# Grice-Lab/HmmUFOtu

Measured on AMD Instinct MI355X. Metric: reads placed/sec (whole node), gg_97_otus GTR+dGamma 250bp; HBM GB/s %peak, higher is better.
Workload: dtype f64

## Files before the change

hmmufotu_amd/csrc/hu_engine.hip:

```cpp
#include <algorithm>
#include <cmath>
#include <cstdio>
#include <cstring>
#include <limits>
#include <map>
#include <atomic>
#include <thread>
#include <memory>
#include <mutex>
#include <chrono>
#include <fstream>
#include <sstream>
#include <new>
#include <stdexcept>
#include "hu_common.h"
#include "hu_kern_sep.h"
#include "hu_kern_align.h"
#include "hu_kern_tree.h"
#include "hu_kern_blk.h"
#include "hu_kern_refsort.h"
#include "hu_kern_rank.h"
#include "hu_kern_anneal.h"
#include "hu_kern_build.h"
#include "hu_kern_otucs.h"
// ... 1112 lines not shown
typedef HuPlaceRec HostPlace;

struct HuKnobs {
	int viterbi_hbm = 0;
	int viterbi_values = 0;
	int viterbi_mode = 0;
	int viterbi_dec1 = 0;
	int vw_diag = 0;
	int viterbi_force_redo = 0;
	int tile_unsorted = 0;
	int pairs32 = 0;
	int topk_fast_min = 16384;
	int topk_general = 0;
	int scan_pairs = 0;
	int streaming_sep = 0;
	int est_unsorted = 0, place_unsorted = 0;
	int xcd_map = 1;
	int est_var = 0, place_var = 0;
	int place_nosplit = 0;
	int place_lds_pad = 0;
	int est_lds_pad = 0;
	int vit_lds_pad = 0;
	int scan_lds_pad = 0;
	int trace = 0;
	int width_split = 1;
	int sort_seq = 0;
	int refsort_wgs = HU_RS_WGS_PER_CU * 256;
	int ref_nofuse = 0;
	int refsort_host = 0;
	int inject_fault = 0;
};
struct HuKnobEntry { const char* name; int HuKnobs::* field; };
static const HuKnobEntry kKnobs[] = {
	{"viterbi_hbm", &HuKnobs::viterbi_hbm}, {"viterbi_values", &HuKnobs::viterbi_values}, {"viterbi_mode", &HuKnobs::viterbi_mode},
	{"viterbi_dec1", &HuKnobs::viterbi_dec1}, {"vw_diag", &HuKnobs::vw_diag}, {"viterbi_force_redo", &HuKnobs::viterbi_force_redo},
	{"pairs32", &HuKnobs::pairs32}, {"tile_unsorted", &HuKnobs::tile_unsorted}, {"topk_fast_min", &HuKnobs::topk_fast_min}, {"scan_pairs", &HuKnobs::scan_pairs}, {"topk_general", &HuKnobs::topk_general}, {"streaming_sep", &HuKnobs::streaming_sep},
	{"est_unsorted", &HuKnobs::est_unsorted}, {"place_unsorted", &HuKnobs::place_unsorted}, {"xcd_map", &HuKnobs::xcd_map},
	{"est_var", &HuKnobs::est_var}, {"place_var", &HuKnobs::place_var}, {"place_nosplit", &HuKnobs::place_nosplit}, {"width_split", &HuKnobs::width_split},
	{"place_lds_pad", &HuKnobs::place_lds_pad}, {"est_lds_pad", &HuKnobs::est_lds_pad}, {"vit_lds_pad", &HuKnobs::vit_lds_pad}, {"scan_lds_pad", &HuKnobs::scan_lds_pad}, {"trace", &HuKnobs::trace}, {"inject_fault", &HuKnobs::inject_fault}, {"refsort_host", &HuKnobs::refsort_host}, {"ref_nofuse", &HuKnobs::ref_nofuse}, {"refsort_wgs", &HuKnobs::refsort_wgs}, {"sort_seq", &HuKnobs::sort_seq},
};
static void knobs_from_env(HuKnobs& k) {
	for(const HuKnobEntry& e : kKnobs) {
		std::string env = "HU_";
		for(const char* c = e.name; *c; ++c) env += (char) toupper(*c);
		const char* v = getenv(env.c_str());
		if(!v) continue;
		char* end = nullptr;
		const long x = strtol(v, &end, 10);
		k.*(e.field) = (end == v) ? 1 : (int) x;
	}
}

enum { ST_NONE = 0, ST_READS = 1, ST_ALIGNED = 2, ST_SEEDED = 3, ST_ESTIMATED = 4, ST_FILTERED = 5, ST_PLACED = 6, ST_FINISHED = 7 };

struct hu_batch {
	hu_db* db = nullptr;
	int maxReads = 0, n = 0, nSeq = 0, state = ST_NONE;
	bool paired = false, fromCodes = false, profile = false;
	HuKnobs knob;
	int maxBases = 1 << 30;
	bool fixedRoot = false;
	bool placesGiven = false;
	bool pair16 = false;
	int scanWidth = 0;
	int pairsKind = 0;
	int seedCap = HU_MAX_SEEDS;
	hipStream_t stream = nullptr;
	hipEvent_t ev[2 * HU_T_COUNT];
	bool evSet[HU_T_COUNT] = {false};
	float ms[HU_T_COUNT];
	double wall[4] = {0, 0, 0, 0};
	DBuf<char> dBases, dTraces, dRows;
	DBuf<HuReadDesc> dDescs;
	DBuf<double> dScratch;
	DBuf<uint8_t> dDec;
	DBuf<HuVitOut> dVit;
	DBuf<HuAlnDev> dAlns;
	DBuf<int8_t> dCodes;
	DBuf<int32_t> dStart, dEnd, dSeedCnt, dSeedId, dGiven, dPermCnt;
	DBuf<uint16_t> dPerm;
	DBuf<uint32_t> dRp, dPairs, dSeedDN, dParDN, dBmin, dRSpan, dTileSpan;
	DBuf<int32_t> dTileQ, dSlotRead, dReadSlot;
	DBuf<uint32_t> dRq;
	DBuf<unsigned long long> dRefScratch;
	DBuf<int32_t> dHv, dZeroPar; DBuf<unsigned long long> dPairsC; int refHvCount = 0; double refHvHeight = NAN;
	DBuf<int32_t> dBail, dNanCnt, dNanId; DBuf<uint32_t> dNanDN;
	int nRefBail = 0;
	DBuf<uint32_t> dRefPiv; DBuf<unsigned long long> dRefL0; bool refFused = false;
	int refHostAll = 0;
	DBuf<int32_t> dIns, dTileIns, dRetry;
	DBuf<uint32_t> dSortK, dSortV;
	DBuf<uint32_t> dCsCnt;
	DBuf<HuEstOut> dEst;
	DBuf<HuCand> dCands;
	DBuf<HuPlaceOut> dPlaceOut;
	DBuf<int32_t> dCandCnt, dCandOff, dMeta;
	DBuf<uint8_t> dFiltSlot;
	DBuf<HuPlaceRec> dPlaces;
	DBuf<hu_place_rec> dBest;
	size_t nc = 0;
	int maxGapSites = 0, maxBaseSites = 0;
	bool hostCands = false;
	DBuf<double> dRootLL;
	PinnedVec<double> hRootLL;
// ... 183 lines not shown
		tr += rd.len + b->db->dev.K + 8;
	}
	int rc;
	if((rc = b->dBases.ensure(b->hBases.size() + 1)) != HU_OK) return rc;
	b->cellsTotal = cells; b->cornerTotal = corners;
	if((rc = b->dDec.ensure((size_t) decs + 1)) != HU_OK) return rc;
	if((rc = b->dTraces.ensure((size_t) tr + 1)) != HU_OK) return rc;
	if((rc = b->dVit.ensure(b->nSeq)) != HU_OK) return rc;
	if(!b->hBases.empty()) HIPCHK(hipMemcpyAsync(b->dBases.p, b->hBases.data(), b->hBases.size(), hipMemcpyHostToDevice, b->stream));
	if((rc = upload_descs(b)) != HU_OK) return rc;
	b->state = ST_READS;
	return HU_OK;
} catch(...) { return hu_catch_all("hu_batch_set_reads"); }

static int ensure_read_buffers(hu_batch* b) {
	const HuDbDev& d = b->db->dev;
	const size_t n = (size_t) b->n;
	const size_t tiles = (n + HU_READ_TILE - 1) / HU_READ_TILE;
	int rc;
	if((rc = b->dCodes.ensure(n * d.csLen)) != HU_OK) return rc;
	if((rc = b->dStart.ensure(n)) != HU_OK) return rc;
	if((rc = b->dEnd.ensure(n)) != HU_OK) return rc;
	if((rc = b->dRp.ensure(tiles * d.WQ * HU_READ_TILE * 16)) != HU_OK) return rc;
	if((rc = b->dTileQ.ensure(tiles * (d.WQ + 1))) != HU_OK) return rc;
	if((rc = b->dSlotRead.ensure(std::max<size_t>(tiles, 1) * HU_READ_TILE)) != HU_OK) return rc;
	if((rc = b->dReadSlot.ensure(std::max<size_t>(n, 1))) != HU_OK) return rc;
	if((rc = b->dRq.ensure(std::max<size_t>(n, 1) * ((d.WQ + 31) / 32))) != HU_OK) return rc;
	if((rc = b->dIns.ensure(std::max<size_t>(n, 1) * (HU_MAX_INS + 1))) != HU_OK) return rc;
	if((rc = b->dTileIns.ensure(std::max<size_t>(tiles, 1) * (HU_READ_TILE * HU_MAX_INS + 1))) != HU_OK) return rc;
	if((rc = b->dRSpan.ensure(std::max<size_t>(n, 1) * 2)) != HU_OK) return rc;
	if((rc = b->dTileSpan.ensure(std::max<size_t>(tiles, 1) * 2)) != HU_OK) return rc;
	return HU_OK;
}

static int order_by_key(hu_batch* b, const uint32_t* key, const uint32_t* val, size_t n, uint32_t bound, uint32_t* out, bool runsInOrder) {
	if(!n) return HU_OK;
	const size_t m = (size_t) bound + 1;
	int rc;
	const size_t nTiles = (m + 1023) / 1024;
	if((rc = b->dCsCnt.ensure(3 * m + nTiles + 8)) != HU_OK) return rc;
	uint32_t* cnt = b->dCsCnt.p; uint32_t* start = cnt + m; uint32_t* cur = start + m + 1; uint32_t* tiles = cur + m;
	HIPCHK(hipMemsetAsync(cnt, 0, m * 4, b->stream));
	k_cs_hist<<<(unsigned)((n + 255) / 256), 256, 0, b->stream>>>((int) n, key, bound, cnt);
	k_cs_tile_sums<<<(unsigned) nTiles, 1024, 0, b->stream>>>((int) m, cnt, tiles);
	k_cs_scan_tiles<<<1, 1024, 0, b->stream>>>((int) nTiles, tiles);
	k_cs_scan<<<(unsigned) nTiles, 1024, 0, b->stream>>>((int) m, cnt, tiles, start, cur);
	k_cs_scatter<<<(unsigned)((n + 255) / 256), 256, 0, b->stream>>>((int) n, key, val, bound, cur, out);
	if(runsInOrder) k_cs_runs<<<(unsigned)((m + 3) / 4), 256, 0, b->stream>>>((int) bound, start, out);
	HIPCHK(hipGetLastError());
	return HU_OK;
}

static int tile_reads(hu_batch* b, const HuAlnDev* alns) {
	const int n = b->n;
	if(!n) return HU_OK;
	const int tiles = (n + HU_READ_TILE - 1) / HU_READ_TILE;
	int rc;
	if((rc = b->dSortK.ensure((size_t) n * 2)) != HU_OK || (rc = b->dSortV.ensure((size_t) n * 2)) != HU_OK) return rc;
	k_tile_keys<<<(n + 255) / 256, 256, 0, b->stream>>>(n, alns, b->dStart.p, b->dEnd.p, b->dSortK.p, b->dSortV.p);
	if(b->knob.tile_unsorted) HIPCHK(hipMemcpyAsync(b->dSortV.p + n, b->dSortV.p, (size_t) n * 4, hipMemcpyDeviceToDevice, b->stream));
	else if((rc = order_by_key(b, b->dSortK.p, b->dSortV.p, (size_t) n, (uint32_t) b->db->dev.csLen + 1u, b->dSortV.p + n, true)) != HU_OK) return rc;
	k_tile_slots<<<(tiles * HU_READ_TILE + 255) / 256, 256, 0, b->stream>>>(n, tiles * HU_READ_TILE, b->dSortV.p + n, b->dSlotRead.p, b->dReadSlot.p);
	HIPCHK(hipGetLastError());
	return HU_OK;
}

static int set_aligned_impl(hu_batch* b, int n, const int8_t* codes, hipMemcpyKind kind, const int32_t* start, const int32_t* end, int maxBases = -1) {
	if(!b || n < 0 || n > b->maxReads || (n > 0 && (!codes || !start || !end))) { hu_set_error("hu_batch_set_aligned: bad argument"); return HU_ERR_ARG; }
	HIPCHK(hipSetDevice(b->db->device));
	const HuDbDev& d = b->db->dev;
	b->n = n; b->nSeq = n; b->paired = false; b->fromCodes = true;
	if(maxBases >= 0) b->maxBases = maxBases;
	else {
		int mb = 0;
		for(int r = 0; r < n; ++r) {
			if(!(start[r] >= 0 && start[r] <= end[r] && end[r] < d.csLen)) continue;
			const int8_t* c = codes + (size_t) r * d.csLen; int k = 0;
			for(int j = start[r]; j <= end[r]; ++j) k += c[j] >= 0;
			mb = std::max(mb, k);
		}
		b->maxBases = mb;
	}
	int rc;
	if((rc = ensure_read_buffers(b)) != HU_OK) return rc;
	b->hAlns.assign(n, HuAlnDev());
	b->hStart.assign(start, start + n); b->hEnd.assign(end, end + n);
	for(int r = 0; r < n; ++r) {
		HuAlnDev& a = b->hAlns[r];
		memset(&a, 0, sizeof(a));
		const bool ok = start[r] >= 0 && start[r] <= end[r] && end[r] < d.csLen && start[r] >= d.winStart && end[r] < d.winStart + d.winLen;
		a.status = ok ? HU_READ_OK : HU_READ_INVALID;
		a.csStart = start[r] + 1; a.csEnd = end[r] + 1;
		if(!ok) { b->hStart[r] = (int32_t) d.winStart; b->hEnd[r] = (int32_t) d.winStart - 1; }
	}
	(void) hipGetLastError();
	if(n) {
		if((const void*) codes != (const void*) b->dCodes.p) HIPCHK(hipMemcpyAsync(b->dCodes.p, codes, (size_t) n * d.csLen, kind, b->stream));
		HIPCHK(hipMemcpyAsync(b->dStart.p, b->hStart.data(), (size_t) n * 4, hipMemcpyHostToDevice, b->stream));
		HIPCHK(hipMemcpyAsync(b->dEnd.p, b->hEnd.data(), (size_t) n * 4, hipMemcpyHostToDevice, b->stream));
		const int tiles = (n + HU_READ_TILE - 1) / HU_READ_TILE;
		HIPCHK(hipMemsetAsync(b->dRp.p, 0, (size_t) tiles * d.WQ * HU_READ_TILE * 16 * 4, b->stream));
		if((rc = tile_reads(b, nullptr)) != HU_OK) return rc;
		k_planes_from_codes<<<n, 64, 0, b->stream>>>(d, b->dCodes.p, b->dStart.p, b->dEnd.p, b->dRp.p, b->dRq.p, b->dIns.p, b->dReadSlot.p, (uint2*) b->dRSpan.p);
		k_tile_lists<<<tiles, 64, 0, b->stream>>>(d, n, b->dRq.p, b->dIns.p, b->dTileQ.p, b->dTileIns.p, b->dSlotRead.p, (const uint2*) b->dRSpan.p, (uint2*) b->dTileSpan.p);
		HIPCHK(hipGetLastError());
	}
	b->state = ST_ALIGNED;
	return HU_OK;
}
extern "C" int hu_batch_set_aligned(hu_batch* b, int n, const int8_t* codes, const int32_t* start, const int32_t* end) try {
	return set_aligned_impl(b, n, codes, hipMemcpyHostToDevice, start, end);
} catch(...) { return hu_catch_all("hu_batch_set_aligned"); }

enum VitFill { VF_WAVE4, VF_WAVE4_DIAG1, VF_WAVE4_DIAG2, VF_WAVE8, VF_DEC2_256, VF_DEC2_512, VF_DEC, VF_VALUES, VF_HBM };
struct VitPlan {
	VitFill fill;
	size_t lds;
	int decRpl;
	bool wave() const { return fill <= VF_WAVE8; }
	bool dec() const { return fill <= VF_DEC; }
};
static VitPlan plan_viterbi(const HuKnobs& kb, int maxLen, size_t vlds, int haloW) {
	if(vlds > 96 * 1024 || kb.viterbi_hbm) return {VF_HBM, 0, 0};
	if(kb.viterbi_values) return {VF_VALUES, vlds, 0};
	const int mode = kb.viterbi_mode ? kb.viterbi_mode : (kb.viterbi_dec1 ? 1 : 0);
	if(mode == 0 && maxLen <= 512) {
		const size_t wl = (size_t) 3 * std::min(haloW, 512) * sizeof(double) + (size_t)(kb.vit_lds_pad > 0 && kb.vit_lds_pad <= 40 ? kb.vit_lds_pad : 0) * 1024;
		if(maxLen > 256) return {VF_WAVE8, wl, 8};
// ... 114 lines not shown
				if((rc = fillValues(b->dDescs.p, b->nSeq, b->dScratch.p, b->dVit.p, HU_READ_NEEDS_VALUES)) != HU_OK) return rc;
				HIPCHK(hipGetLastError());
				HIPCHK(hipMemcpyAsync(b->hVit.data(), b->dVit.p, (size_t) b->nSeq * sizeof(HuVitOut), hipMemcpyDeviceToHost, b->stream));
				HIPCHK(hu_wait(b->stream));
			}
		}
		std::vector<int> redo;
		for(int s = 0; s < b->nSeq; ++s) if(b->hVit[s].status == HU_READ_NEEDS_FULL && !(b->hDescs[s].nRegions == 1 && !b->hDescs[s].reg[0].band)) redo.push_back(s);
		auto fullDp = [&](HuReadDesc& rd) { build_regions(b->db, rd.len, nullptr, rd); return rd.scratchOff; };
		if((rc = redoChunked(redo, fullDp, 0)) != HU_OK) return rc;
		for(int s : redo) b->hDescs[s].nRegions = -1;
		if(kb.trace) {
			static const char* const fillName[] = {"k_viterbi_wave<4>", "k_viterbi_wave<4, 1>", "k_viterbi_wave<4, 2>", "k_viterbi_wave<8>", "k_viterbi_dec2<256>", "k_viterbi_dec2<512>", "k_viterbi_dec", "k_viterbi_lds", "k_viterbi"};
			fprintf(stderr, "[hu] align: %d sequences, longest %d, fill %s, %zu bytes of LDS, %zu redone for values, %zu by the full-DP fallback\n", b->nSeq, maxLen, fillName[vp.fill], vp.lds, nValues, redo.size());
		}
		for(int s = 0; s < b->nSeq; ++s) if(b->hVit[s].status == HU_READ_NEEDS_FULL) { b->hVit[s].status = HU_READ_INVALID; hostVit = true; }
		if(hostVit) HIPCHK(hipMemcpyAsync(b->dVit.p, b->hVit.data(), (size_t) b->nSeq * sizeof(HuVitOut), hipMemcpyHostToDevice, b->stream));
		{
			Timer t(b, HU_T_ALIGN_BUILD);
			k_align_rows<<<b->nSeq, 64, 0, b->stream>>>(d, b->dDescs.p, b->dBases.p, b->dTraces.p, b->dVit.p, b->dRows.p, b->dAlns.p);
			if(b->paired) k_merge_rows<<<b->n, 256, 0, b->stream>>>(d, b->n, o->ignore_orient, b->dRows.p, b->dAlns.p);
			const int tiles = (b->n + HU_READ_TILE - 1) / HU_READ_TILE;
			HIPCHK(hipMemsetAsync(b->dRp.p, 0, (size_t) tiles * d.WQ * HU_READ_TILE * 16 * 4, b->stream));
			if((rc = tile_reads(b, b->dAlns.p)) != HU_OK) return rc;
			k_encode_rows<<<b->n, 64, 0, b->stream>>>(d, b->dRows.p, b->dAlns.p, b->dCodes.p, b->dStart.p, b->dEnd.p, b->dRp.p, b->dRq.p, b->dIns.p, b->dReadSlot.p, (uint2*) b->dRSpan.p);
			k_tile_lists<<<tiles, 64, 0, b->stream>>>(d, b->n, b->dRq.p, b->dIns.p, b->dTileQ.p, b->dTileIns.p, b->dSlotRead.p, (const uint2*) b->dRSpan.p, (uint2*) b->dTileSpan.p);
		}
		HIPCHK(hipGetLastError());
		b->hAlns.resize(b->nSeq);
		b->hStart.resize(b->n); b->hEnd.resize(b->n);
		HIPCHK(hipMemcpyAsync(b->hAlns.data(), b->dAlns.p, (size_t) b->nSeq * sizeof(HuAlnDev), hipMemcpyDeviceToHost, b->stream));
		HIPCHK(hipMemcpyAsync(b->hStart.data(), b->dStart.p, (size_t) b->n * 4, hipMemcpyDeviceToHost, b->stream));
		HIPCHK(hipMemcpyAsync(b->hEnd.data(), b->dEnd.p, (size_t) b->n * 4, hipMemcpyDeviceToHost, b->stream));
		HIPCHK(hu_wait(b->stream));
		for(int s = 0; s < b->nSeq; ++s) b->hAlns[s].usedFull |= (b->hDescs[s].nRegions == -1 || (b->hDescs[s].nRegions == 1 && !b->hDescs[s].reg[0].band)) ? 1 : 0;
	}
	b->state = ST_ALIGNED;
	return HU_OK;
} catch(...) { return hu_catch_all("hu_align_batch"); }

__global__ void k_seed_drop_empty(int n, const int32_t* __restrict__ rstart, const int32_t* __restrict__ rend, int32_t* __restrict__ seedCnt);
static inline HuReadPlanes read_planes(const hu_batch* b) { return HuReadPlanes{b->dRp.p, b->dRq.p, b->dIns.p, b->dReadSlot.p, (const uint2*) b->dRSpan.p}; }


extern "C" int hu_sort_desc_device(int device, const double* keys, int rows, int n, int32_t* order) try {
	if(!keys || !order || rows < 1 || n < 0 || n > HU_MAX_SEEDS) { hu_set_error("hu_sort_desc_device: bad argument"); return HU_ERR_ARG; }
	if(hu_device_count() <= 0) { hu_set_error("no gfx950 device visible: the engine has no CPU path"); return HU_ERR_DEVICE; }
	HIPCHK(hipSetDevice(device));
	if(n == 0) return HU_OK;
	DBuf<double> dk; DBuf<int32_t> dor;
	int rc;
// ... 361 lines not shown
	uint32_t* bmin = nullptr;
	if(dOnly) {
		if((rc = b->dBmin.ensure(std::max<size_t>(n, 1) * nBlk + 16)) != HU_OK) return rc;
		if((rc = b->dRetry.ensure(n + 1)) != HU_OK) return rc;
		bmin = b->dBmin.p;
	}
	b->refFused = refOrder && n > 0 && ref_fused_l0(b, o, b->pair16);
	if(b->refFused) {
		if((rc = b->dRefPiv.ensure(n * 4)) != HU_OK || (rc = b->dRefL0.ensure(n * (size_t)(d.nNodesPad / 64) * 2)) != HU_OK) return rc;
		k_ref_pivots<<<(unsigned)((n + 63) / 64), 64, 0, b->stream>>>(d, read_planes(b), b->n, b->dRefPiv.p);
		HIPCHK(hipGetLastError());
	}
	uint32_t* stat = bmin && b->knob.trace ? bmin + n * nBlk : nullptr;
	if(stat) HIPCHK(hipMemsetAsync(stat, 0, 64, b->stream));
	(void) hipGetLastError();
	if(n) {
		const int tiles = (b->n + HU_READ_TILE - 1) / HU_READ_TILE;
		const dim3 grid(tiles, d.nNodesPad / 256);
		{
			Timer t(b, HU_T_SEED_PDIST);
			const dim3 grid4(tiles, (d.nNodesPad + 1023) / 1024);
			if(dOnly && narrow) k_seed_dscan4<uint8_t><<<grid4, 256, (size_t)(b->knob.scan_lds_pad > 0 && b->knob.scan_lds_pad <= 44 ? b->knob.scan_lds_pad : 0) * 1024, b->stream>>>(d, b->dRp.p, b->dTileQ.p, (uint8_t*) b->dPairs.p, b->dSlotRead.p, bmin, (const uint2*) b->dTileSpan.p);
			else if(dOnly) k_seed_dscan4<uint16_t><<<grid4, 256, 0, b->stream>>>(d, b->dRp.p, b->dTileQ.p, (uint16_t*) b->dPairs.p, b->dSlotRead.p, bmin, (const uint2*) b->dTileSpan.p);
			else if(b->refFused && b->pair16) k_seed_pdist2<uint16_t, true><<<grid, 256, 0, b->stream>>>(d, b->dRp.p, b->dTileQ.p, b->dTileIns.p, (uint16_t*) b->dPairs.p, b->dSlotRead.p, b->dRefPiv.p, b->dRefL0.p);
			else if(b->refFused) k_seed_pdist2<uint32_t, true><<<grid, 256, 0, b->stream>>>(d, b->dRp.p, b->dTileQ.p, b->dTileIns.p, b->dPairs.p, b->dSlotRead.p, b->dRefPiv.p, b->dRefL0.p);
			else if(b->pair16) k_seed_pdist2<uint16_t><<<grid, 256, 0, b->stream>>>(d, b->dRp.p, b->dTileQ.p, b->dTileIns.p, (uint16_t*) b->dPairs.p, b->dSlotRead.p);
			else k_seed_pdist2<uint32_t><<<grid, 256, 0, b->stream>>>(d, b->dRp.p, b->dTileQ.p, b->dTileIns.p, b->dPairs.p, b->dSlotRead.p);
		}
		{
			Timer t(b, HU_T_SEED_TOPK);
			if(dOnly) {
				int32_t* retry = b->dRetry.p;
				HIPCHK(hipMemsetAsync(retry, 0, 4, b->stream));
				#define TOPK_ARGS(T) d, (const T*) b->dPairs.p, bmin, read_planes(b), o->max_nseed, b->dSeedCnt.p, b->dSeedId.p, b->dSeedDN.p, b->dParDN.p, stat, retry
				if(narrow) { k_seed_topk_straight<uint8_t><<<b->n, 256, 0, b->stream>>>(TOPK_ARGS(uint8_t), b->knob.topk_general); k_seed_topk_d<uint8_t, true><<<std::min(b->n, 1024), 256, 0, b->stream>>>(TOPK_ARGS(uint8_t)); }
				else { k_seed_topk_straight<uint16_t><<<b->n, 256, 0, b->stream>>>(TOPK_ARGS(uint16_t), b->knob.topk_general); k_seed_topk_d<uint16_t, true><<<std::min(b->n, 1024), 256, 0, b->stream>>>(TOPK_ARGS(uint16_t)); }
				#undef TOPK_ARGS
			}
			else if(refOrder) { if((rc = seed_order_libstdcxx_device(b, o)) != HU_OK) return rc; }
			else {
				if(b->pair16) k_seed_topk<uint16_t><<<b->n, 256, 0, b->stream>>>(d, (const uint16_t*) b->dPairs.p, o->max_height, o->max_nseed, b->dSeedCnt.p, b->dSeedId.p, b->dSeedDN.p, b->knob.topk_fast_min);
				else k_seed_topk<uint32_t><<<b->n, 256, 0, b->stream>>>(d, b->dPairs.p, o->max_height, o->max_nseed, b->dSeedCnt.p, b->dSeedId.p, b->dSeedDN.p, b->knob.topk_fast_min);
				k_parent_pairs<<<((unsigned) n * HU_MAX_SEEDS + 255) / 256, 256, 0, b->stream>>>(d, b->n, b->dPairs.p, b->pair16 ? 1 : 0, b->dSeedCnt.p, b->dSeedId.p, b->dParDN.p);
			}
		}
		k_seed_drop_empty<<<(b->n + 255) / 256, 256, 0, b->stream>>>(b->n, b->dStart.p, b->dEnd.p, b->dSeedCnt.p);
		HIPCHK(hipGetLastError());
		if(stat) {
			uint32_t h[16];
			HIPCHK(hipMemcpyAsync(h, stat, 64, hipMemcpyDeviceToHost, b->stream)); HIPCHK(hu_wait(b->stream));
// ... 1233 lines not shown
```

hmmufotu_amd/csrc/hu_kern_align.h:

```cpp
#pragma once
#include "hu_common.h"

struct HuVitOut { int32_t alnStart, alnEnd, alnFrom, alnTo, traceLen, status; double minScore; };

__device__ inline bool reg_contains(const HuRegion& g, int i, int j) {
	if(j < g.j0 || j > g.j1 || i < g.i0 || i > g.i1) return false;
	if(g.band) { int dist = (i - g.from) - (j - g.start); if(!(dist <= g.nIns && dist >= -g.nDel)) return false; }
	return true;
}

struct VitCtx {
	const HuReadDesc* rd;
	const double* scr;
	double tNN, tNB;
};

__device__ inline void vit_lookup(const VitCtx& c, int upto, int i, int j, double& m, double& ii, double& d) {
	const HuReadDesc& rd = *c.rd;
	for(int r = upto - 1; r >= 0; --r) {
		const HuRegion& g = rd.reg[r];
		if(reg_contains(g, i, j)) {
			const int64_t idx = (g.off + (int64_t)(j - g.j0) * (g.i1 - g.i0 + 1) + (i - g.i0)) * 3;
			m = c.scr[idx]; ii = c.scr[idx + 1]; d = c.scr[idx + 2];
			return;
// ... 996 lines not shown
		}
		ok = (st == HU_READ_OK);
		if(ok) {
			if(b.seqStart < a.seqStart) a.seqStart = b.seqStart;
			if(b.seqEnd > a.seqEnd) a.seqEnd = b.seqEnd;
			if(b.hmmStart < a.hmmStart) a.hmmStart = b.hmmStart;
			if(b.hmmEnd > a.hmmEnd) a.hmmEnd = b.hmmEnd;
			if(b.csStart < a.csStart) a.csStart = b.csStart;
			if(b.csEnd > a.csEnd) a.csEnd = b.csEnd;
			a.cost = a.cost + b.cost;
			a.usedFull |= b.usedFull;
		}
		a.status = st;
		alns[r] = a;
	}
	__syncthreads();
	if(!ok) return;
	char* ra = rows + (size_t) r * db.csLen;
	const char* rb = rows + (size_t)(n + r) * db.csLen;
	for(int c = threadIdx.x; c < db.csLen; c += 256) if(ra[c] == '.' && rb[c] != '.') ra[c] = rb[c];
}

__device__ inline void planes_of_codes(const HuDbDev& db, const int8_t* __restrict__ cd, int start, int end, int r, int slot, int lane,
		uint32_t* __restrict__ rp, uint32_t* __restrict__ rq, int32_t* __restrict__ ins, uint2* __restrict__ rspan) {
	const int tile = slot / HU_READ_TILE, t = slot % HU_READ_TILE;
	const int nw32 = (db.WQ + 31) / 32;
	uint32_t* qbits = rq + (size_t) r * nw32;
	int32_t* il = ins + (size_t) r * (HU_MAX_INS + 1);
	const int QM = (db.K + 127) / 128;
	int nIns = 0;
	for(int base = QM * 128; base < db.WQ * 128; base += 64) {
		const int c = db.posCol[base + lane];
		const bool in = c >= start && c <= end && cd[c >= 0 ? c : 0] >= 0 && c >= 0;
		nIns += __popcll(__ballot(in));
	}
	const bool dense = nIns > HU_MAX_INS;
	uint32_t acc = 0;
	int li = 0;
	uint32_t f1 = 0xffffu, l1 = 0, f2 = 0xffffu, l2 = 0; bool any1 = false, any2 = false;
	for(int base = 0; base < db.WQ * 128; base += 64) {
		const int c = db.posCol[base + lane];
		const int8_t code = c >= 0 ? cd[c] : (int8_t) -2;
		const bool in = c >= start && c <= end && code >= 0;
		const int q = base / 128, w = (base % 128) / 32;
		const bool asList = q >= QM && !dense;
		unsigned long long b0 = __ballot(in && (code & 1)), b1 = __ballot(in && (code & 2)), bv = __ballot(in);
		if(lane == 0 && bv) {
			const uint32_t lo = (uint32_t) base + (uint32_t)(__ffsll((long long) bv) - 1), hi = (uint32_t) base + 63u - (uint32_t) __clzll((long long) bv);
			if(q < QM) { if(!any1) { f1 = lo; any1 = true; } l1 = hi; }
			else { if(!any2) { f2 = lo; any2 = true; } l2 = hi; }
		}
		if(lane == 0) {
			if(asList) {
				unsigned long long m = bv;
				while(m) { const int bit = __ffsll((long long) m) - 1; m &= m - 1; il[1 + li++] = ((base + bit) << 2) | (int)(((b0 >> bit) & 1) | (((b1 >> bit) & 1) << 1)); }
				b0 = b1 = bv = 0;
			}
			uint32_t* dst = rp + (((size_t) tile * db.WQ + q) * HU_READ_TILE + t) * 16;
			dst[0 + w] = (uint32_t) b0; dst[0 + w + 1] = (uint32_t)(b0 >> 32);
			dst[4 + w] = (uint32_t) b1; dst[4 + w + 1] = (uint32_t)(b1 >> 32);
			dst[8 + w] = (uint32_t) bv; dst[8 + w + 1] = (uint32_t)(bv >> 32);
			if(bv) acc |= 1u << (q & 31);
			if((q & 31) == 31 && w == 2) { qbits[q >> 5] = acc; acc = 0; }
		}
	}
	if(lane == 0) {
		if(db.WQ & 31) qbits[(db.WQ - 1) >> 5] = acc; il[0] = li;
		rspan[r] = make_uint2((any1 ? f1 : 0xffffu) | ((any1 ? l1 : 0u) << 16), (any2 ? f2 : 0xffffu) | ((any2 ? l2 : 0u) << 16));
	}
}

__global__ __launch_bounds__(64) void k_encode_rows(HuDbDev db, const char* __restrict__ rows, HuAlnDev* __restrict__ alns,
		int8_t* __restrict__ codes, int32_t* __restrict__ rstart, int32_t* __restrict__ rend, uint32_t* __restrict__ rp, uint32_t* __restrict__ rq,
		int32_t* __restrict__ ins, const int32_t* __restrict__ readSlot, uint2* __restrict__ rspan) {
	const int r = blockIdx.x, lane = threadIdx.x;
	const HuAlnDev a = alns[r];
	const char* row = rows + (size_t) r * db.csLen;
	int8_t* cd = codes + (size_t) r * db.csLen;
	bool ok = a.status == HU_READ_OK;
	if(ok && (a.csStart - 1 < db.winStart || a.csEnd - 1 >= db.winStart + db.winLen)) {
		ok = false;
		if(lane == 0) alns[r].status = HU_READ_OUT_OF_WINDOW;
	}
	const int start = ok ? a.csStart - 1 : (int) db.winStart, end = ok ? a.csEnd - 1 : (int) db.winStart - 1;
	if(lane == 0) { rstart[r] = start; rend[r] = end; }
	for(int c = lane; c < db.csLen; c += 64) {
		char ch = row[c];
		if(ch >= 'a' && ch <= 'z') ch = (char)(ch - 32);
		cd[c] = c_sym_map[(int) ch & 127];
	}
	__syncthreads();
	planes_of_codes(db, cd, start, end, r, readSlot[r], lane, rp, rq, ins, rspan);
}

__global__ __launch_bounds__(64) void k_planes_from_codes(HuDbDev db, const int8_t* __restrict__ codes,
		const int32_t* __restrict__ rstart, const int32_t* __restrict__ rend, uint32_t* __restrict__ rp, uint32_t* __restrict__ rq,
		int32_t* __restrict__ ins, const int32_t* __restrict__ readSlot, uint2* __restrict__ rspan) {
	const int r = blockIdx.x, lane = threadIdx.x;
	planes_of_codes(db, codes + (size_t) r * db.csLen, rstart[r], rend[r], r, readSlot[r], lane, rp, rq, ins, rspan);
}

__global__ void k_tile_keys(int n, const HuAlnDev* __restrict__ alns, const int32_t* __restrict__ rstart, const int32_t* __restrict__ rend,
		uint32_t* __restrict__ key, uint32_t* __restrict__ val) {
	const int r = blockIdx.x * 256 + threadIdx.x;
	if(r >= n) return;
	uint32_t k;
	if(alns) k = alns[r].status == HU_READ_OK ? (uint32_t) alns[r].csStart : 0x7fffffffu;
	else k = rend[r] >= rstart[r] ? (uint32_t) rstart[r] + 1u : 0x7fffffffu;
	key[r] = k; val[r] = (uint32_t) r;
}
__global__ void k_tile_slots(int n, int nSlots, const uint32_t* __restrict__ sortedRead, int32_t* __restrict__ slotRead, int32_t* __restrict__ readSlot) {
	const int s = blockIdx.x * 256 + threadIdx.x;
	if(s >= nSlots) return;
	if(s < n) { const int r = (int) sortedRead[s]; slotRead[s] = r; readSlot[r] = s; }
	else slotRead[s] = -1;
}

__global__ __launch_bounds__(64) void k_tile_lists(HuDbDev db, int n, const uint32_t* __restrict__ rq, const int32_t* __restrict__ ins,
		int32_t* __restrict__ tileQ, int32_t* __restrict__ tileIns, const int32_t* __restrict__ slotRead, const uint2* __restrict__ rspan, uint2* __restrict__ tileSpan) {
	const int tile = blockIdx.x, lane = threadIdx.x;
	const int nw32 = (db.WQ + 31) / 32;
	int32_t* out = tileQ + (size_t) tile * (db.WQ + 1);
	int cnt = 0;
	for(int w = 0; w < nw32; ++w) {
		uint32_t m = 0;
		if(lane < HU_READ_TILE) { const int r = slotRead[tile * HU_READ_TILE + lane]; if(r >= 0) m = rq[(size_t) r * nw32 + w]; }
		for(int s = 32; s > 0; s >>= 1) m |= __shfl_xor(m, s);
		if(lane == 0) while(m) { const int b = __ffs(m) - 1; m &= m - 1; out[1 + cnt++] = w * 32 + b; }
	}
	if(lane == 0) {
		out[0] = cnt;
		int32_t* til = tileIns + (size_t) tile * (HU_READ_TILE * HU_MAX_INS + 1);
		int ne = 0;
		for(int t = 0; t < HU_READ_TILE; ++t) {
			const int r = slotRead[tile * HU_READ_TILE + t];
			if(r < 0) continue;
			const int32_t* il = ins + (size_t) r * (HU_MAX_INS + 1);
			for(int e = 0; e < il[0]; ++e) til[1 + ne++] = (t << 24) | il[1 + e];
		}
		til[0] = ne;
		uint32_t f1 = 0xffffu, l1 = 0, f2 = 0xffffu, l2 = 0; bool a1 = false, a2 = false;
		for(int t = 0; t < HU_READ_TILE; ++t) {
			const int r = slotRead[tile * HU_READ_TILE + t];
			if(r < 0) continue;
			const uint2 s2 = rspan[r];
			if((s2.x & 0xffffu) <= (s2.x >> 16)) { f1 = a1 ? min(f1, s2.x & 0xffffu) : (s2.x & 0xffffu); l1 = a1 ? max(l1, s2.x >> 16) : (s2.x >> 16); a1 = true; }
			if((s2.y & 0xffffu) <= (s2.y >> 16)) { f2 = a2 ? min(f2, s2.y & 0xffffu) : (s2.y & 0xffffu); l2 = a2 ? max(l2, s2.y >> 16) : (s2.y >> 16); a2 = true; }
		}
		tileSpan[tile] = make_uint2((a1 ? f1 : 0xffffu) | ((a1 ? l1 : 0u) << 16), (a2 ? f2 : 0xffffu) | ((a2 ? l2 : 0u) << 16));
	}
}
// ... 1 lines not shown
```

hmmufotu_amd/csrc/hu_kern_sep.h:

```cpp
#pragma once
#include "hu_common.h"

#define HU_TOPK_BINS 4097
#define HU_TOPK_CAP 4096

template<class PT> struct HuPair;
template<> struct HuPair<uint32_t> {
	static constexpr int PPV = 4;
	__device__ static inline uint32_t canon(uint32_t x) { return x; }
	__device__ static inline uint32_t pack(uint32_t c) { return c; }
	__device__ static inline void unpack(const uint4& v, uint32_t* o) { o[0] = v.x; o[1] = v.y; o[2] = v.z; o[3] = v.w; }
};
template<> struct HuPair<uint16_t> {
	static constexpr int PPV = 8;
	__device__ static inline uint32_t canon(uint32_t x) { return ((x >> 8) << 16) | (x & 0xffu); }
	__device__ static inline uint16_t pack(uint32_t c) { return (uint16_t)(((c >> 16) << 8) | (c & 0xffu)); }
	__device__ static inline void unpack(const uint4& v, uint32_t* o) {
		const uint32_t w[4] = {v.x, v.y, v.z, v.w};
#pragma unroll
		for(int e = 0; e < 8; ++e) o[e] = canon((w[e >> 1] >> ((e & 1) * 16)) & 0xffffu);
	}
};
__device__ inline uint32_t hu_pair_load(const void* pairs, size_t idx, int p16) {
	return p16 ? HuPair<uint16_t>::canon(((const uint16_t*) pairs)[idx]) : ((const uint32_t*) pairs)[idx];
// ... 19 lines not shown
	uint32_t f1 = 0xffffu, l1 = 0, f2 = 0xffffu, l2 = 0; bool any1 = false, any2 = false;
	for(int q = 0; q < db.WQ; ++q) {
		const uint4 v = db.planes[((size_t) q * 3 + 2) * db.nNodesPad + node];
		const uint32_t w[4] = {v.x, v.y, v.z, v.w};
		for(int k = 0; k < 4; ++k) {
			if(!w[k]) continue;
			const uint32_t lo = (uint32_t) q * 128 + k * 32 + (__ffs(w[k]) - 1), hi = (uint32_t) q * 128 + k * 32 + 31 - __clz(w[k]);
			if(q < db.QM) { if(!any1) { f1 = lo; any1 = true; } l1 = hi; }
			else { if(!any2) { f2 = lo; any2 = true; } l2 = hi; }
		}
	}
	cover[node] = make_uint2((any1 ? f1 : 0xffffu) | ((any1 ? l1 : 0u) << 16), (any2 ? f2 : 0xffffu) | ((any2 ? l2 : 0u) << 16));
}
__device__ inline bool hu_span_meets(uint32_t a, uint32_t b) {
	return (a & 0xffffu) <= (b >> 16) && (b & 0xffffu) <= (a >> 16) && (a & 0xffffu) <= (a >> 16) && (b & 0xffffu) <= (b >> 16);
}
__device__ inline bool hu_cover_meets(uint2 node, uint2 read) { return hu_span_meets(node.x, read.x) || hu_span_meets(node.y, read.y); }

template<int CTRL>
__device__ inline uint32_t dpp_min_full(uint32_t v) {
	const uint32_t o = (uint32_t) __builtin_amdgcn_mov_dpp((int) v, CTRL, 0xf, 0xf, true);
	return o < v ? o : v;
}
template<class PT, bool L0 = false>
__global__ __launch_bounds__(256) void k_seed_pdist2(HuDbDev db, const uint32_t* __restrict__ rp,
		const int32_t* __restrict__ tileQ, const int32_t* __restrict__ tileIns, PT* __restrict__ pairs, const int32_t* __restrict__ slotRead,
		uint32_t* __restrict__ piv = nullptr, unsigned long long* __restrict__ l0m = nullptr) {
	constexpr int T = HU_READ_TILE;
	__shared__ uint32_t acc[T][256];
	const int tile = blockIdx.x, tid = threadIdx.x;
	const int node = blockIdx.y * 256 + tid;
	const int32_t* __restrict__ ql = tileQ + (size_t) tile * (db.WQ + 1);
	const int32_t* __restrict__ til = tileIns + (size_t) tile * (T * HU_MAX_INS + 1);
	const int nq = ql[0], ne = til[0];
	uint32_t d[T], N[T];
#pragma unroll
	for(int t = 0; t < T; ++t) { d[t] = 0; N[t] = 0; }
	if(ne) {
#pragma unroll
		for(int t = 0; t < T; ++t) acc[t][tid] = 0;
	}
	const size_t np = (size_t) db.nNodesPad;
	for(int qi = 0; qi < nq; ++qi) {
		const int q = ql[1 + qi];
		const uint4 n0 = db.planes[((size_t) q * 3 + 0) * np + node], n1 = db.planes[((size_t) q * 3 + 1) * np + node], nv = db.planes[((size_t) q * 3 + 2) * np + node];
		const uint32_t* __restrict__ r = rp + (((size_t) tile * db.WQ + q) * T) * 16;
#pragma unroll
		for(int t = 0; t < T; ++t) {
			const uint32_t* rt = r + t * 16;
			uint32_t k, x;
			k = nv.x & rt[8];  x = ((n0.x ^ rt[0]) | (n1.x ^ rt[4])) & k; d[t] += __popc(x); N[t] += __popc(k);
			k = nv.y & rt[9];  x = ((n0.y ^ rt[1]) | (n1.y ^ rt[5])) & k; d[t] += __popc(x); N[t] += __popc(k);
			k = nv.z & rt[10]; x = ((n0.z ^ rt[2]) | (n1.z ^ rt[6])) & k; d[t] += __popc(x); N[t] += __popc(k);
			k = nv.w & rt[11]; x = ((n0.w ^ rt[3]) | (n1.w ^ rt[7])) & k; d[t] += __popc(x); N[t] += __popc(k);
		}
	}
	{
		const size_t npw = np / 64;
		const int nb = __builtin_amdgcn_readfirstlane(node >> 6), lane = tid & 63;
		for(int e = 0; e < ne; ++e) {
			const int ent = til[1 + e];
			const int t = ent >> 24, pos = (ent >> 2) & 0x3fffff, code = ent & 3;
			const unsigned long long* cp = db.colPlanes + ((size_t)(pos - db.QM * 128) * 3) * npw + nb;
			const unsigned long long W0 = cp[0], W1 = cp[npw], Wv = cp[2 * npw];
			const uint32_t valid = (uint32_t)(Wv >> lane) & 1u, nc = ((uint32_t)(W0 >> lane) & 1u) | (((uint32_t)(W1 >> lane) & 1u) << 1);
			const uint32_t add = valid | ((valid & (nc != (uint32_t) code ? 1u : 0u)) << 16);
			atomicAdd(&acc[t][tid], add);
		}
	}
	const bool counts = L0 && node < db.nNodes && node != db.root;
	bool zero = false;
#pragma unroll
	for(int t = 0; t < T; ++t) {
		const int read = slotRead[tile * T + t];
		if(read >= 0) {
			const uint32_t v = ((d[t] << 16) | N[t]) + (ne ? acc[t][tid] : 0u);
			pairs[(size_t) read * np + node] = HuPair<PT>::pack(v);
			if(L0) {
// ... 17 lines not shown
}

template<class DT>
__global__ __launch_bounds__(256, 3) void k_seed_dscan4(HuDbDev db, const uint32_t* __restrict__ rp,
		const int32_t* __restrict__ tileQ, DT* __restrict__ dm, const int32_t* __restrict__ slotRead, uint32_t* __restrict__ bminD, const uint2* __restrict__ tileSpan) {
	constexpr int T = HU_READ_TILE, M = 4;
	constexpr uint32_t DMAX = (uint32_t)(DT) ~(DT) 0;
	static_assert(T == 16, "sixteen reads x sixteen dwords per quad = one dword per thread");
	__shared__ __attribute__((aligned(16))) uint32_t rpl2[2][T * 16];
	__shared__ __attribute__((aligned(16))) uint32_t mb[4][T][64];
	const int tile = blockIdx.x, tid = threadIdx.x, lane = tid & 63, wave = tid >> 6;
	const int node0 = blockIdx.y * (256 * M) + tid * M;
	const bool live = node0 < db.nNodesPad;
	const int nl = live ? node0 : 0;
	const int32_t* __restrict__ ql = tileQ + (size_t) tile * (db.WQ + 1);
	const int nq = ql[0];
	uint32_t d[T][M];
#pragma unroll
	for(int t = 0; t < T; ++t)
#pragma unroll
		for(int m = 0; m < M; ++m) d[t][m] = 0;
	const size_t np = (size_t) db.nNodesPad;
	for(int qi = 0; qi < nq; ++qi) {
		const int q = ql[1 + qi];
		const uint32_t mine = rp[((size_t) tile * db.WQ + q) * (T * 16) + tid];
		uint4 n0[M], n1[M], nv[M];
#pragma unroll
		for(int m = 0; m < M; ++m) {
			n0[m] = db.planes[((size_t) q * 3 + 0) * np + nl + m]; n1[m] = db.planes[((size_t) q * 3 + 1) * np + nl + m]; nv[m] = db.planes[((size_t) q * 3 + 2) * np + nl + m];
		}
		uint32_t* rpl = rpl2[qi & 1];
		rpl[tid] = mine;
		__syncthreads();
		uint4 r0 = *reinterpret_cast<const uint4*>(&rpl[0]), r1 = *reinterpret_cast<const uint4*>(&rpl[4]), rv = *reinterpret_cast<const uint4*>(&rpl[8]);
#pragma unroll
		for(int t = 0; t < T; ++t) {
			const int tn = t + 1 < T ? t + 1 : t;
			const uint4 p0 = *reinterpret_cast<const uint4*>(&rpl[tn * 16]), p1 = *reinterpret_cast<const uint4*>(&rpl[tn * 16 + 4]), pv = *reinterpret_cast<const uint4*>(&rpl[tn * 16 + 8]);
			uint32_t a[M][4];
#pragma unroll
			for(int m = 0; m < M; ++m) { a[m][0] = n0[m].x ^ r0.x; a[m][1] = n0[m].y ^ r0.y; a[m][2] = n0[m].z ^ r0.z; a[m][3] = n0[m].w ^ r0.w; }
			__builtin_amdgcn_sched_barrier(0);
#pragma unroll
			for(int m = 0; m < M; ++m) {
				a[m][0] = __builtin_amdgcn_bitop3_b32(a[m][0], n1[m].x, r1.x, 0xf6); a[m][1] = __builtin_amdgcn_bitop3_b32(a[m][1], n1[m].y, r1.y, 0xf6);
				a[m][2] = __builtin_amdgcn_bitop3_b32(a[m][2], n1[m].z, r1.z, 0xf6); a[m][3] = __builtin_amdgcn_bitop3_b32(a[m][3], n1[m].w, r1.w, 0xf6);
			}
// ... 1258 lines not shown
```

Measured before the change: 380,800.

## Add word-major read plane layout and skip dead words in pdist2 scan

A second read-plane buffer is written in a word-major, read-contiguous layout (three planes × 16 reads per 32-bit word), so the pdist2 kernel can load each word's reads as 16-wide vectors. The tile-list kernel now records, for each quad, which of its four words carries any valid bits for the tile, packed into the high bits of the quad index. pdist2 skips words with no live bits, and dscan4 masks off the new bits. This saves loads and popcounts on sparse quads, at the cost of an extra buffer, an extra memset and more writes during encoding. A trace knob can report how many words are dead.

```diff
diff --git a/hmmufotu_amd/csrc/hu_engine.hip b/hmmufotu_amd/csrc/hu_engine.hip
--- a/hmmufotu_amd/csrc/hu_engine.hip
+++ b/hmmufotu_amd/csrc/hu_engine.hip
@@ -1158,6 +1158,7 @@
 	int est_lds_pad = 0;
 	int vit_lds_pad = 0;
 	int scan_lds_pad = 0;
+	int scan_words = 1;
 	int trace = 0;
 	int width_split = 1;
 	int sort_seq = 0;
@@ -1173,7 +1174,7 @@
 	{"pairs32", &HuKnobs::pairs32}, {"tile_unsorted", &HuKnobs::tile_unsorted}, {"topk_fast_min", &HuKnobs::topk_fast_min}, {"scan_pairs", &HuKnobs::scan_pairs}, {"topk_general", &HuKnobs::topk_general}, {"streaming_sep", &HuKnobs::streaming_sep},
 	{"est_unsorted", &HuKnobs::est_unsorted}, {"place_unsorted", &HuKnobs::place_unsorted}, {"xcd_map", &HuKnobs::xcd_map},
 	{"est_var", &HuKnobs::est_var}, {"place_var", &HuKnobs::place_var}, {"place_nosplit", &HuKnobs::place_nosplit}, {"width_split", &HuKnobs::width_split},
-	{"place_lds_pad", &HuKnobs::place_lds_pad}, {"est_lds_pad", &HuKnobs::est_lds_pad}, {"vit_lds_pad", &HuKnobs::vit_lds_pad}, {"scan_lds_pad", &HuKnobs::scan_lds_pad}, {"trace", &HuKnobs::trace}, {"inject_fault", &HuKnobs::inject_fault}, {"refsort_host", &HuKnobs::refsort_host}, {"ref_nofuse", &HuKnobs::ref_nofuse}, {"refsort_wgs", &HuKnobs::refsort_wgs}, {"sort_seq", &HuKnobs::sort_seq},
+	{"place_lds_pad", &HuKnobs::place_lds_pad}, {"est_lds_pad", &HuKnobs::est_lds_pad}, {"vit_lds_pad", &HuKnobs::vit_lds_pad}, {"scan_lds_pad", &HuKnobs::scan_lds_pad}, {"scan_words", &HuKnobs::scan_words}, {"trace", &HuKnobs::trace}, {"inject_fault", &HuKnobs::inject_fault}, {"refsort_host", &HuKnobs::refsort_host}, {"ref_nofuse", &HuKnobs::ref_nofuse}, {"refsort_wgs", &HuKnobs::refsort_wgs}, {"sort_seq", &HuKnobs::sort_seq},
 };
 static void knobs_from_env(HuKnobs& k) {
 	for(const HuKnobEntry& e : kKnobs) {
@@ -1215,7 +1216,7 @@
 	DBuf<int8_t> dCodes;
 	DBuf<int32_t> dStart, dEnd, dSeedCnt, dSeedId, dGiven, dPermCnt;
 	DBuf<uint16_t> dPerm;
-	DBuf<uint32_t> dRp, dPairs, dSeedDN, dParDN, dBmin, dRSpan, dTileSpan;
+	DBuf<uint32_t> dRp, dRpw, dPairs, dSeedDN, dParDN, dBmin, dRSpan, dTileSpan;
 	DBuf<int32_t> dTileQ, dSlotRead, dReadSlot;
 	DBuf<uint32_t> dRq;
 	DBuf<unsigned long long> dRefScratch;
@@ -1445,6 +1446,7 @@
 	if((rc = b->dStart.ensure(n)) != HU_OK) return rc;
 	if((rc = b->dEnd.ensure(n)) != HU_OK) return rc;
 	if((rc = b->dRp.ensure(tiles * d.WQ * HU_READ_TILE * 16)) != HU_OK) return rc;
+	if((rc = b->dRpw.ensure(tiles * d.WQ * HU_READ_TILE * 12)) != HU_OK) return rc;
 	if((rc = b->dTileQ.ensure(tiles * (d.WQ + 1))) != HU_OK) return rc;
 	if((rc = b->dSlotRead.ensure(std::max<size_t>(tiles, 1) * HU_READ_TILE)) != HU_OK) return rc;
 	if((rc = b->dReadSlot.ensure(std::max<size_t>(n, 1))) != HU_OK) return rc;
@@ -1488,6 +1490,16 @@
 	return HU_OK;
 }
 
+static int trace_tile_words(hu_batch* b, int tiles) {
+	const int WQ = b->db->dev.WQ;
+	std::vector<int32_t> tq((size_t) tiles * (WQ + 1));
+	HIPCHK(hipMemcpyAsync(tq.data(), b->dTileQ.p, tq.size() * 4, hipMemcpyDeviceToHost, b->stream));
+	HIPCHK(hu_wait(b->stream));
+	long quads = 0, live = 0;
+	for(int t = 0; t < tiles; ++t) for(int i = 0; i < tq[(size_t) t * (WQ + 1)]; ++i) { ++quads; live += __builtin_popcount((uint32_t) tq[(size_t) t * (WQ + 1) + 1 + i] >> 16); }
+	fprintf(stderr, "[hu] scan tiles: %d tiles, %.2f words in listed quads and %.2f live words per tile (%.1f %% dead)\n", tiles, 4.0 * quads / std::max(tiles, 1), (double) live / std::max(tiles, 1), quads ? 100.0 - 25.0 * live / quads : 0.0);
+	return HU_OK;
+}
 static int set_aligned_impl(hu_batch* b, int n, const int8_t* codes, hipMemcpyKind kind, const int32_t* start, const int32_t* end, int maxBases = -1) {
 	if(!b || n < 0 || n > b->maxReads || (n > 0 && (!codes || !start || !end))) { hu_set_error("hu_batch_set_aligned: bad argument"); return HU_ERR_ARG; }
 	HIPCHK(hipSetDevice(b->db->device));
@@ -1523,10 +1535,12 @@
 		HIPCHK(hipMemcpyAsync(b->dEnd.p, b->hEnd.data(), (size_t) n * 4, hipMemcpyHostToDevice, b->stream));
 		const int tiles = (n + HU_READ_TILE - 1) / HU_READ_TILE;
 		HIPCHK(hipMemsetAsync(b->dRp.p, 0, (size_t) tiles * d.WQ * HU_READ_TILE * 16 * 4, b->stream));
+			HIPCHK(hipMemsetAsync(b->dRpw.p, 0, (size_t) tiles * d.WQ * HU_READ_TILE * 12 * 4, b->stream));
 		if((rc = tile_reads(b, nullptr)) != HU_OK) return rc;
-		k_planes_from_codes<<<n, 64, 0, b->stream>>>(d, b->dCodes.p, b->dStart.p, b->dEnd.p, b->dRp.p, b->dRq.p, b->dIns.p, b->dReadSlot.p, (uint2*) b->dRSpan.p);
-		k_tile_lists<<<tiles, 64, 0, b->stream>>>(d, n, b->dRq.p, b->dIns.p, b->dTileQ.p, b->dTileIns.p, b->dSlotRead.p, (const uint2*) b->dRSpan.p, (uint2*) b->dTileSpan.p);
+		k_planes_from_codes<<<n, 64, 0, b->stream>>>(d, b->dCodes.p, b->dStart.p, b->dEnd.p, b->dRp.p, b->dRpw.p, b->dRq.p, b->dIns.p, b->dReadSlot.p, (uint2*) b->dRSpan.p);
+		k_tile_lists<<<tiles, 64, 0, b->stream>>>(d, n, b->dRq.p, b->dIns.p, b->dTileQ.p, b->dTileIns.p, b->dSlotRead.p, (const uint2*) b->dRSpan.p, (uint2*) b->dTileSpan.p, b->dRp.p, b->knob.scan_words);
 		HIPCHK(hipGetLastError());
+		if(b->knob.trace && (rc = trace_tile_words(b, tiles)) != HU_OK) return rc;
 	}
 	b->state = ST_ALIGNED;
 	return HU_OK;
@@ -1687,11 +1701,13 @@
 			if(b->paired) k_merge_rows<<<b->n, 256, 0, b->stream>>>(d, b->n, o->ignore_orient, b->dRows.p, b->dAlns.p);
 			const int tiles = (b->n + HU_READ_TILE - 1) / HU_READ_TILE;
 			HIPCHK(hipMemsetAsync(b->dRp.p, 0, (size_t) tiles * d.WQ * HU_READ_TILE * 16 * 4, b->stream));
+			HIPCHK(hipMemsetAsync(b->dRpw.p, 0, (size_t) tiles * d.WQ * HU_READ_TILE * 12 * 4, b->stream));
 			if((rc = tile_reads(b, b->dAlns.p)) != HU_OK) return rc;
-			k_encode_rows<<<b->n, 64, 0, b->stream>>>(d, b->dRows.p, b->dAlns.p, b->dCodes.p, b->dStart.p, b->dEnd.p, b->dRp.p, b->dRq.p, b->dIns.p, b->dReadSlot.p, (uint2*) b->dRSpan.p);
-			k_tile_lists<<<tiles, 64, 0, b->stream>>>(d, b->n, b->dRq.p, b->dIns.p, b->dTileQ.p, b->dTileIns.p, b->dSlotRead.p, (const uint2*) b->dRSpan.p, (uint2*) b->dTileSpan.p);
+			k_encode_rows<<<b->n, 64, 0, b->stream>>>(d, b->dRows.p, b->dAlns.p, b->dCodes.p, b->dStart.p, b->dEnd.p, b->dRp.p, b->dRpw.p, b->dRq.p, b->dIns.p, b->dReadSlot.p, (uint2*) b->dRSpan.p);
+			k_tile_lists<<<tiles, 64, 0, b->stream>>>(d, b->n, b->dRq.p, b->dIns.p, b->dTileQ.p, b->dTileIns.p, b->dSlotRead.p, (const uint2*) b->dRSpan.p, (uint2*) b->dTileSpan.p, b->dRp.p, kb.scan_words);
 		}
 		HIPCHK(hipGetLastError());
+		if(kb.trace && (rc = trace_tile_words(b, (b->n + HU_READ_TILE - 1) / HU_READ_TILE)) != HU_OK) return rc;
 		b->hAlns.resize(b->nSeq);
 		b->hStart.resize(b->n); b->hEnd.resize(b->n);
 		HIPCHK(hipMemcpyAsync(b->hAlns.data(), b->dAlns.p, (size_t) b->nSeq * sizeof(HuAlnDev), hipMemcpyDeviceToHost, b->stream));
@@ -2099,10 +2115,10 @@
 			const dim3 grid4(tiles, (d.nNodesPad + 1023) / 1024);
 			if(dOnly && narrow) k_seed_dscan4<uint8_t><<<grid4, 256, (size_t)(b->knob.scan_lds_pad > 0 && b->knob.scan_lds_pad <= 44 ? b->knob.scan_lds_pad : 0) * 1024, b->stream>>>(d, b->dRp.p, b->dTileQ.p, (uint8_t*) b->dPairs.p, b->dSlotRead.p, bmin, (const uint2*) b->dTileSpan.p);
 			else if(dOnly) k_seed_dscan4<uint16_t><<<grid4, 256, 0, b->stream>>>(d, b->dRp.p, b->dTileQ.p, (uint16_t*) b->dPairs.p, b->dSlotRead.p, bmin, (const uint2*) b->dTileSpan.p);
-			else if(b->refFused && b->pair16) k_seed_pdist2<uint16_t, true><<<grid, 256, 0, b->stream>>>(d, b->dRp.p, b->dTileQ.p, b->dTileIns.p, (uint16_t*) b->dPairs.p, b->dSlotRead.p, b->dRefPiv.p, b->dRefL0.p);
-			else if(b->refFused) k_seed_pdist2<uint32_t, true><<<grid, 256, 0, b->stream>>>(d, b->dRp.p, b->dTileQ.p, b->dTileIns.p, b->dPairs.p, b->dSlotRead.p, b->dRefPiv.p, b->dRefL0.p);
-			else if(b->pair16) k_seed_pdist2<uint16_t><<<grid, 256, 0, b->stream>>>(d, b->dRp.p, b->dTileQ.p, b->dTileIns.p, (uint16_t*) b->dPairs.p, b->dSlotRead.p);
-			else k_seed_pdist2<uint32_t><<<grid, 256, 0, b->stream>>>(d, b->dRp.p, b->dTileQ.p, b->dTileIns.p, b->dPairs.p, b->dSlotRead.p);
+			else if(b->refFused && b->pair16) k_seed_pdist2<uint16_t, true><<<grid, 256, 0, b->stream>>>(d, b->dRpw.p, b->dTileQ.p, b->dTileIns.p, (uint16_t*) b->dPairs.p, b->dSlotRead.p, b->dRefPiv.p, b->dRefL0.p);
+			else if(b->refFused) k_seed_pdist2<uint32_t, true><<<grid, 256, 0, b->stream>>>(d, b->dRpw.p, b->dTileQ.p, b->dTileIns.p, b->dPairs.p, b->dSlotRead.p, b->dRefPiv.p, b->dRefL0.p);
+			else if(b->pair16) k_seed_pdist2<uint16_t><<<grid, 256, 0, b->stream>>>(d, b->dRpw.p, b->dTileQ.p, b->dTileIns.p, (uint16_t*) b->dPairs.p, b->dSlotRead.p);
+			else k_seed_pdist2<uint32_t><<<grid, 256, 0, b->stream>>>(d, b->dRpw.p, b->dTileQ.p, b->dTileIns.p, b->dPairs.p, b->dSlotRead.p);
 		}
 		{
 			Timer t(b, HU_T_SEED_TOPK);
diff --git a/hmmufotu_amd/csrc/hu_kern_align.h b/hmmufotu_amd/csrc/hu_kern_align.h
--- a/hmmufotu_amd/csrc/hu_kern_align.h
+++ b/hmmufotu_amd/csrc/hu_kern_align.h
@@ -1042,7 +1042,7 @@
 }
 
 __device__ inline void planes_of_codes(const HuDbDev& db, const int8_t* __restrict__ cd, int start, int end, int r, int slot, int lane,
-		uint32_t* __restrict__ rp, uint32_t* __restrict__ rq, int32_t* __restrict__ ins, uint2* __restrict__ rspan) {
+		uint32_t* __restrict__ rp, uint32_t* __restrict__ rpw, uint32_t* __restrict__ rq, int32_t* __restrict__ ins, uint2* __restrict__ rspan) {
 	const int tile = slot / HU_READ_TILE, t = slot % HU_READ_TILE;
 	const int nw32 = (db.WQ + 31) / 32;
 	uint32_t* qbits = rq + (size_t) r * nw32;
@@ -1080,6 +1080,10 @@
 			dst[0 + w] = (uint32_t) b0; dst[0 + w + 1] = (uint32_t)(b0 >> 32);
 			dst[4 + w] = (uint32_t) b1; dst[4 + w + 1] = (uint32_t)(b1 >> 32);
 			dst[8 + w] = (uint32_t) bv; dst[8 + w + 1] = (uint32_t)(bv >> 32);
+			uint32_t* dw = rpw + ((((size_t) tile * db.WQ + q) * 4 + w) * 3) * HU_READ_TILE + t;
+			dw[0 * HU_READ_TILE] = (uint32_t) b0; dw[3 * HU_READ_TILE] = (uint32_t)(b0 >> 32);
+			dw[1 * HU_READ_TILE] = (uint32_t) b1; dw[4 * HU_READ_TILE] = (uint32_t)(b1 >> 32);
+			dw[2 * HU_READ_TILE] = (uint32_t) bv; dw[5 * HU_READ_TILE] = (uint32_t)(bv >> 32);
 			if(bv) acc |= 1u << (q & 31);
 			if((q & 31) == 31 && w == 2) { qbits[q >> 5] = acc; acc = 0; }
 		}
@@ -1091,7 +1095,7 @@
 }
 
 __global__ __launch_bounds__(64) void k_encode_rows(HuDbDev db, const char* __restrict__ rows, HuAlnDev* __restrict__ alns,
-		int8_t* __restrict__ codes, int32_t* __restrict__ rstart, int32_t* __restrict__ rend, uint32_t* __restrict__ rp, uint32_t* __restrict__ rq,
+		int8_t* __restrict__ codes, int32_t* __restrict__ rstart, int32_t* __restrict__ rend, uint32_t* __restrict__ rp, uint32_t* __restrict__ rpw, uint32_t* __restrict__ rq,
 		int32_t* __restrict__ ins, const int32_t* __restrict__ readSlot, uint2* __restrict__ rspan) {
 	const int r = blockIdx.x, lane = threadIdx.x;
 	const HuAlnDev a = alns[r];
@@ -1110,14 +1114,14 @@
 		cd[c] = c_sym_map[(int) ch & 127];
 	}
 	__syncthreads();
-	planes_of_codes(db, cd, start, end, r, readSlot[r], lane, rp, rq, ins, rspan);
+	planes_of_codes(db, cd, start, end, r, readSlot[r], lane, rp, rpw, rq, ins, rspan);
 }
 
 __global__ __launch_bounds__(64) void k_planes_from_codes(HuDbDev db, const int8_t* __restrict__ codes,
-		const int32_t* __restrict__ rstart, const int32_t* __restrict__ rend, uint32_t* __restrict__ rp, uint32_t* __restrict__ rq,
+		const int32_t* __restrict__ rstart, const int32_t* __restrict__ rend, uint32_t* __restrict__ rp, uint32_t* __restrict__ rpw, uint32_t* __restrict__ rq,
 		int32_t* __restrict__ ins, const int32_t* __restrict__ readSlot, uint2* __restrict__ rspan) {
 	const int r = blockIdx.x, lane = threadIdx.x;
-	planes_of_codes(db, codes + (size_t) r * db.csLen, rstart[r], rend[r], r, readSlot[r], lane, rp, rq, ins, rspan);
+	planes_of_codes(db, codes + (size_t) r * db.csLen, rstart[r], rend[r], r, readSlot[r], lane, rp, rpw, rq, ins, rspan);
 }
 
 __global__ void k_tile_keys(int n, const HuAlnDev* __restrict__ alns, const int32_t* __restrict__ rstart, const int32_t* __restrict__ rend,
@@ -1137,7 +1141,8 @@
 }
 
 __global__ __launch_bounds__(64) void k_tile_lists(HuDbDev db, int n, const uint32_t* __restrict__ rq, const int32_t* __restrict__ ins,
-		int32_t* __restrict__ tileQ, int32_t* __restrict__ tileIns, const int32_t* __restrict__ slotRead, const uint2* __restrict__ rspan, uint2* __restrict__ tileSpan) {
+		int32_t* __restrict__ tileQ, int32_t* __restrict__ tileIns, const int32_t* __restrict__ slotRead, const uint2* __restrict__ rspan, uint2* __restrict__ tileSpan,
+		const uint32_t* __restrict__ rp, int words) {
 	const int tile = blockIdx.x, lane = threadIdx.x;
 	const int nw32 = (db.WQ + 31) / 32;
 	int32_t* out = tileQ + (size_t) tile * (db.WQ + 1);
@@ -1146,7 +1151,13 @@
 		uint32_t m = 0;
 		if(lane < HU_READ_TILE) { const int r = slotRead[tile * HU_READ_TILE + lane]; if(r >= 0) m = rq[(size_t) r * nw32 + w]; }
 		for(int s = 32; s > 0; s >>= 1) m |= __shfl_xor(m, s);
-		if(lane == 0) while(m) { const int b = __ffs(m) - 1; m &= m - 1; out[1 + cnt++] = w * 32 + b; }
+		while(m) {
+			const int q = w * 32 + __ffs(m) - 1; m &= m - 1;
+			unsigned long long live = __ballot(rp[(((size_t) tile * db.WQ + q) * HU_READ_TILE + (lane >> 2)) * 16 + 8 + (lane & 3)] != 0u);
+			live |= live >> 32; live |= live >> 16; live |= live >> 8; live |= live >> 4;
+			if(lane == 0) out[1 + cnt] = q | (int32_t)((words ? (uint32_t) live & 15u : 15u) << 16);
+			++cnt;
+		}
 	}
 	if(lane == 0) {
 		out[0] = cnt;
diff --git a/hmmufotu_amd/csrc/hu_kern_sep.h b/hmmufotu_amd/csrc/hu_kern_sep.h
--- a/hmmufotu_amd/csrc/hu_kern_sep.h
+++ b/hmmufotu_amd/csrc/hu_kern_sep.h
@@ -65,8 +65,9 @@
 	const uint32_t o = (uint32_t) __builtin_amdgcn_mov_dpp((int) v, CTRL, 0xf, 0xf, true);
 	return o < v ? o : v;
 }
+typedef uint32_t HuU32x16 __attribute__((ext_vector_type(16)));
 template<class PT, bool L0 = false>
-__global__ __launch_bounds__(256) void k_seed_pdist2(HuDbDev db, const uint32_t* __restrict__ rp,
+__global__ __launch_bounds__(256) void k_seed_pdist2(HuDbDev db, const uint32_t* __restrict__ rpw,
 		const int32_t* __restrict__ tileQ, const int32_t* __restrict__ tileIns, PT* __restrict__ pairs, const int32_t* __restrict__ slotRead,
 		uint32_t* __restrict__ piv = nullptr, unsigned long long* __restrict__ l0m = nullptr) {
 	constexpr int T = HU_READ_TILE;
@@ -85,18 +86,20 @@
 	}
 	const size_t np = (size_t) db.nNodesPad;
 	for(int qi = 0; qi < nq; ++qi) {
-		const int q = ql[1 + qi];
+		const int qe = ql[1 + qi], q = qe & 0xffff, live = qe >> 16;
 		const uint4 n0 = db.planes[((size_t) q * 3 + 0) * np + node], n1 = db.planes[((size_t) q * 3 + 1) * np + node], nv = db.planes[((size_t) q * 3 + 2) * np + node];
-		const uint32_t* __restrict__ r = rp + (((size_t) tile * db.WQ + q) * T) * 16;
-#pragma unroll
-		for(int t = 0; t < T; ++t) {
-			const uint32_t* rt = r + t * 16;
-			uint32_t k, x;
-			k = nv.x & rt[8];  x = ((n0.x ^ rt[0]) | (n1.x ^ rt[4])) & k; d[t] += __popc(x); N[t] += __popc(k);
-			k = nv.y & rt[9];  x = ((n0.y ^ rt[1]) | (n1.y ^ rt[5])) & k; d[t] += __popc(x); N[t] += __popc(k);
-			k = nv.z & rt[10]; x = ((n0.z ^ rt[2]) | (n1.z ^ rt[6])) & k; d[t] += __popc(x); N[t] += __popc(k);
-			k = nv.w & rt[11]; x = ((n0.w ^ rt[3]) | (n1.w ^ rt[7])) & k; d[t] += __popc(x); N[t] += __popc(k);
-		}
+		const uint32_t* __restrict__ r = rpw + (((size_t) tile * db.WQ + q) * 4) * (3 * T);
+#define HU_SCAN_WORD(W, C) \
+		if(live & (1 << W)) { \
+			const HuU32x16* rw = reinterpret_cast<const HuU32x16*>(r + W * (3 * T)); \
+			const HuU32x16 r0 = rw[0], r1 = rw[1], rv = rw[2]; \
+			_Pragma("unroll") \
+			for(int t = 0; t < T; ++t) { \
+				const uint32_t k = nv.C & rv[t], x = ((n0.C ^ r0[t]) | (n1.C ^ r1[t])) & k; d[t] += __popc(x); N[t] += __popc(k); \
+			} \
+		}
+		HU_SCAN_WORD(0, x) HU_SCAN_WORD(1, y) HU_SCAN_WORD(2, z) HU_SCAN_WORD(3, w)
+#undef HU_SCAN_WORD
 	}
 	{
 		const size_t npw = np / 64;
@@ -160,7 +163,7 @@
 		for(int m = 0; m < M; ++m) d[t][m] = 0;
 	const size_t np = (size_t) db.nNodesPad;
 	for(int qi = 0; qi < nq; ++qi) {
-		const int q = ql[1 + qi];
+		const int q = ql[1 + qi] & 0xffff;
 		const uint32_t mine = rp[((size_t) tile * db.WQ + q) * (T * 16) + tid];
 		uint4 n0[M], n1[M], nv[M];
 #pragma unroll
```

Measured after the change: 371,300. 2.5% lower.
